# octavian-ganea/equidock_public

Hardware: NVIDIA H100
Metric: protein_pairs_per_sec_iegmn_fwd_kabsch (higher is better)
Workload: dtype f32

## Files before the change

### equidock_public_b200/csrc/attn_tc.cu

```cuda
#include "tc_common.cuh"

namespace eqd {

#define AT_THREADS 256
#define AT_KEYS 64
#define AT_CHUNK_BYTES 8192
#define AT_A_SPLIT 16384
#define AT_LD 68

struct AtGroupSmem {
  unsigned char k[2][3][AT_CHUNK_BYTES];
  unsigned char v[2][3][AT_CHUNK_BYTES];
  float red[EQD_TM * 2];
  float x5c[2][AT_KEYS * 16];
  float red5[EQD_TM * 2 * 5];
};
struct AtSmem {
  unsigned char qa[3 * AT_A_SPLIT];
  unsigned char pa[3 * AT_A_SPLIT];
  AtGroupSmem grp;
  unsigned long long k_bar[2], v_bar[2];
};

__global__ void __launch_bounds__(AT_THREADS, 1)
attention0_tc_kernel(eqd_graph g, const float* __restrict__ proj, int pw, const unsigned char* __restrict__ kv,
                    long kv_split_stride, const float* __restrict__ x5, float* __restrict__ mu, int ldmu) {
  extern __shared__ __align__(128) unsigned char smem_raw[];
  AtSmem& S = *reinterpret_cast<AtSmem*>(smem_raw);
  const int tid = threadIdx.x, q = tid, half = q >> 7, r = q & 127, wgi = tid >> 7;
  AtGroupSmem& G = S.grp;
  if (tid == 0) {
    for (int b = 0; b < 2; ++b) {
      mbar_init(&S.k_bar[b], 1);
      mbar_init(&S.v_bar[b], 1);
    }
    asm volatile("fence.mbarrier_init.release.cluster;" ::: "memory");
  }
  __syncthreads();
  const unsigned k_saddr = smem_u32(G.k), v_saddr = smem_u32(G.v);
  const unsigned qa_saddr = smem_u32(S.qa), pa_saddr = smem_u32(S.pa);
  float* const dtile = reinterpret_cast<float*>(S.pa);
  unsigned kph[2] = {0, 0}, vph[2] = {0, 0};
  const int B = g.n_pairs;
  const unsigned char* k_g = kv;
  const unsigned char* v_g = kv + 3 * kv_split_stride;

  auto load_chunk = [&](const unsigned char* src, unsigned char (*dst)[AT_CHUNK_BYTES], unsigned long long* bar, int blk0,
                        int x5buf) {
    if (q == 0) {
      const bool with5 = x5buf >= 0;
      mbar_expect_tx(bar, 3 * AT_CHUNK_BYTES + (with5 ? AT_KEYS * 64 : 0));
#pragma unroll
      for (int s = 0; s < 3; ++s) bulk_g2s(dst[s], src + s * kv_split_stride + (long)blk0 * 1024, AT_CHUNK_BYTES, bar);
      if (with5) bulk_g2s(G.x5c[x5buf], x5 + (long)blk0 * 8 * 16, AT_KEYS * 64, bar);
    }
  };
  auto add_s5 = [&](float (&s)[32], const float* xc, const float (&q5)[5]) {
#pragma unroll
    for (int i = 0; i < 32; ++i) {
      const float* row = xc + (half * 32 + i) * 16;
      const float4 k4 = *reinterpret_cast<const float4*>(row);
      const float k8 = row[8];
      s[i] += q5[0] * k4.x + q5[1] * k4.y + q5[2] * k4.z + q5[3] * k4.w + q5[4] * k8;
    }
  };
  auto gemm_s = [&](int kb_, bool hi_only) {
    float d[32];
    wg_gemm6<64>(d, [&](int sp, int kb) { return a_desc_at<EQD_TM>(qa_saddr, AT_A_SPLIT, wgi, sp, kb); },
                 [&](int sp, int kk) { return b_desc_ex(k_saddr + (kb_ * 3 + sp) * AT_CHUNK_BYTES + kk * 256, 128, 1024); },
                 4, false, hi_only);
    wg_store_d<64>(dtile + wgi * 64 * AT_LD, AT_LD, d, tid & 127);
  };
  auto gemm_pv = [&](int vb_) {
    float d[32];
    wg_gemm6<64, 1>(d, [&](int sp, int kb) { return a_desc_at<EQD_TM>(pa_saddr, AT_A_SPLIT, wgi, sp, kb); },
                    [&](int sp, int kk) { return b_desc_ex(v_saddr + (vb_ * 3 + sp) * AT_CHUNK_BYTES + kk * 2048, 1024, 128); },
                    4, false);
    __syncthreads();
    wg_store_d<64>(dtile + wgi * 64 * AT_LD, AT_LD, d, tid & 127);
  };

  for (int tile = blockIdx.x; tile < g.n_node_tiles; tile += gridDim.x) {
    const int seg = g.node_tiles[2 * tile], node0 = g.node_tiles[2 * tile + 1];
    const int nvalid = min(EQD_TM, g.seg_ptr[seg + 1] - node0);
    const int pseg = seg < B ? seg + B : seg - B;
    const int j0 = g.seg_ptr[pseg], j1 = g.seg_ptr[pseg + 1];
    const int blk_lo = j0 >> 3, blk_hi = (j1 + 7) >> 3;
    const int nchunks = (blk_hi - blk_lo + 7) >> 3;
    const int node = node0 + r;
    const bool valid = r < nvalid;
    if (nchunks > 0) load_chunk(k_g, G.k[0], &S.k_bar[0], blk_lo, 0);
    float q5[5] = {0.f, 0.f, 0.f, 0.f, 0.f};
    if (valid) {
#pragma unroll
      for (int e = 0; e < 5; ++e) q5[e] = x5[(long)node * 16 + 10 + e];
    }
    {
      float v[32];
      const float4* sp = reinterpret_cast<const float4*>(proj + (long)node * pw + 128 + half * 32);
#pragma unroll
      for (int c4 = 0; c4 < 8; ++c4) {
        float4 t = valid ? sp[c4] : make_float4(0.f, 0.f, 0.f, 0.f);
        v[c4 * 4] = t.x; v[c4 * 4 + 1] = t.y; v[c4 * 4 + 2] = t.z; v[c4 * 4 + 3] = t.w;
      }
      store_half_split3<EQD_TM>(S.qa, AT_A_SPLIT, r, half * 32, v);
    }
    tc_fence_before();
    __syncthreads();
    float mx = -INFINITY;
    for (int c = 0; c < nchunks; ++c) {
      const int kb_ = c & 1;
      mbar_wait(&S.k_bar[kb_], kph[kb_]);
      kph[kb_] ^= 1;
      if (c + 1 < nchunks) load_chunk(k_g, G.k[kb_ ^ 1], &S.k_bar[kb_ ^ 1], blk_lo + 8 * (c + 1), kb_ ^ 1);
      else load_chunk(k_g, G.k[kb_ ^ 1], &S.k_bar[kb_ ^ 1], blk_lo, kb_ ^ 1);
      gemm_s(kb_, true);
      __syncthreads();
      float s[32];
      tile_ld32f(dtile, AT_LD, r, half * 32, s);
      add_s5(s, G.x5c[kb_], q5);
      const int key0 = (blk_lo + 8 * c) * 8 + half * 32;
#pragma unroll
      for (int i = 0; i < 32; ++i) {
        int kn = key0 + i;
        mx = fmaxf(mx, (kn >= j0 && kn < j1) ? s[i] : -INFINITY);
      }
      __syncthreads();
    }
    G.red[r * 2 + half] = mx;
    __syncthreads();
    mx = fmaxf(G.red[r * 2], G.red[r * 2 + 1]);
    float l = 0.f;
    float o_acc[32];
#pragma unroll
    for (int i = 0; i < 32; ++i) o_acc[i] = 0.f;
    if (nchunks > 0) load_chunk(v_g, G.v[0], &S.v_bar[0], blk_lo, -1);
    float o5[5] = {0.f, 0.f, 0.f, 0.f, 0.f};
    for (int c = 0; c < nchunks; ++c) {
      const int kb_ = (nchunks + c) & 1, vb_ = c & 1;
      mbar_wait(&S.k_bar[kb_], kph[kb_]);
      kph[kb_] ^= 1;
      if (c + 1 < nchunks) {
        load_chunk(k_g, G.k[kb_ ^ 1], &S.k_bar[kb_ ^ 1], blk_lo + 8 * (c + 1), kb_ ^ 1);
        load_chunk(v_g, G.v[vb_ ^ 1], &S.v_bar[vb_ ^ 1], blk_lo + 8 * (c + 1), -1);
      }
      gemm_s(kb_, false);
      __syncthreads();
      float s[32];
      tile_ld32f(dtile, AT_LD, r, half * 32, s);
      add_s5(s, G.x5c[kb_], q5);
      const int key0 = (blk_lo + 8 * c) * 8 + half * 32;
      float l4[4] = {0.f, 0.f, 0.f, 0.f};
#pragma unroll
      for (int i = 0; i < 32; ++i) {
        int kn = key0 + i;
        float pj = (kn >= j0 && kn < j1) ? expf(s[i] - mx) : 0.f;
        s[i] = pj;
        l4[i & 3] += pj;
        {
          const float* row = G.x5c[kb_] + (half * 32 + i) * 16;
          const float4 v4 = *reinterpret_cast<const float4*>(row + 4);
          o5[0] = fmaf(pj, v4.x, o5[0]);
          o5[1] = fmaf(pj, v4.y, o5[1]);
          o5[2] = fmaf(pj, v4.z, o5[2]);
          o5[3] = fmaf(pj, v4.w, o5[3]);
          o5[4] = fmaf(pj, row[9], o5[4]);
        }
      }
      l += (l4[0] + l4[1]) + (l4[2] + l4[3]);
      __syncthreads();
      store_half_split3<EQD_TM>(S.pa, AT_A_SPLIT, r, half * 32, s);
      tc_fence_before();
      __syncthreads();
      mbar_wait(&S.v_bar[vb_], vph[vb_]);
      vph[vb_] ^= 1;
      gemm_pv(vb_);
      __syncthreads();
      {
        float oc[32];
        tile_ld32f(dtile, AT_LD, r, half * 32, oc);
#pragma unroll
        for (int i = 0; i < 32; ++i) o_acc[i] += oc[i];
      }
      __syncthreads();
    }
    G.red[r * 2 + half] = l;
    {
#pragma unroll
      for (int e = 0; e < 5; ++e) G.red5[(r * 2 + half) * 5 + e] = o5[e];
    }
    __syncthreads();
    l = G.red[r * 2] + G.red[r * 2 + 1];
    {
      const float inv = l > 0.f ? 1.f / l : 0.f;
      if (valid && half == 0) {
        float e8[8];
#pragma unroll
        for (int e = 0; e < 5; ++e) e8[e] = (G.red5[r * 10 + e] + G.red5[r * 10 + 5 + e]) * inv;
        e8[5] = e8[6] = e8[7] = 0.f;
        float4* de = reinterpret_cast<float4*>(mu + (long)node * ldmu + 64);
        de[0] = make_float4(e8[0], e8[1], e8[2], e8[3]);
        de[1] = make_float4(e8[4], e8[5], e8[6], e8[7]);
      }
      if (valid) {
        float4* dst = reinterpret_cast<float4*>(mu + (long)node * ldmu + half * 32);
#pragma unroll
        for (int c4 = 0; c4 < 8; ++c4)
          dst[c4] = make_float4(o_acc[c4 * 4] * inv, o_acc[c4 * 4 + 1] * inv, o_acc[c4 * 4 + 2] * inv, o_acc[c4 * 4 + 3] * inv);
      }
    }
    __syncthreads();
  }
}

#define AT_CHAINS 2

struct __align__(128) AtChainSmem {
  unsigned char k[2][3][AT_CHUNK_BYTES];
  unsigned char v[2][3][AT_CHUNK_BYTES];
  float qs[64 * 64];
  unsigned long long k_bar[2], v_bar[2];
};

struct AtTile {
  int node0, nvalid;
  int j0, j1;
  int blk_lo, nchunks;
};

template <int P>
__global__ void __launch_bounds__(AT_CHAINS * 128, 1)
attention64_tc_kernel(eqd_graph g, const float* __restrict__ proj, const unsigned char* __restrict__ kv,
                      long kv_split_stride, float* __restrict__ mu) {
  extern __shared__ __align__(128) unsigned char smem_raw[];
  AtChainSmem& W = reinterpret_cast<AtChainSmem*>(smem_raw)[threadIdx.x >> 7];
  const int tid = threadIdx.x, wgi = tid >> 7, t = tid & 127, lane = t & 31;
  const int bar = 1 + wgi;
  if (t == 0) {
    for (int b = 0; b < 2; ++b) {
      mbar_init(&W.k_bar[b], 1);
      mbar_init(&W.v_bar[b], 1);
    }
    asm volatile("fence.mbarrier_init.release.cluster;" ::: "memory");
  }
  wg_barrier(bar);
  const unsigned k_saddr = smem_u32(W.k), v_saddr = smem_u32(W.v);
  const int B = g.n_pairs, nht = 2 * g.n_node_tiles, hstride = gridDim.x * AT_CHAINS;
  const unsigned char* k_g = kv;
  const unsigned char* v_g = kv + 3 * kv_split_stride;

  const int chain = blockIdx.x * AT_CHAINS + wgi;
  auto find_tile = [&](int k, AtTile& m) {
    for (; chain + k * hstride < nht; ++k) {
      const int ht = (chain + k * hstride) ^ (k & 1);
      const int seg = __ldg(g.node_tiles + 2 * (ht >> 1));
      m.node0 = __ldg(g.node_tiles + 2 * (ht >> 1) + 1) + 64 * (ht & 1);
      m.nvalid = min(64, __ldg(g.seg_ptr + seg + 1) - m.node0);
      if (m.nvalid <= 0) continue;
      const int pseg = seg < B ? seg + B : seg - B;
      m.j0 = __ldg(g.seg_ptr + pseg);
      m.j1 = __ldg(g.seg_ptr + pseg + 1);
      m.blk_lo = m.j0 >> 3;
      m.nchunks = (((m.j1 + 7) >> 3) - m.blk_lo + 7) >> 3;
      return k;
    }
    return -1;
  };
  unsigned kfill = 0, kcons = 0, vfill = 0, vcons = 0;
  auto fill = [&](unsigned char (*dst)[3][AT_CHUNK_BYTES], unsigned long long* bars, unsigned& n, const unsigned char* src,
                  int blk0) {
    if (t == 0) {
      unsigned long long* b = &bars[n & 1];
      mbar_expect_tx(b, 3 * AT_CHUNK_BYTES);
#pragma unroll
      for (int s = 0; s < 3; ++s) bulk_g2s(dst[n & 1][s], src + s * kv_split_stride + (long)blk0 * 1024, AT_CHUNK_BYTES, b);
    }
    ++n;
  };
  auto consume = [&](unsigned long long* bars, unsigned& n) {
    mbar_wait(&bars[n & 1], (n >> 1) & 1);
    return (int)((n++) & 1);
  };
  auto stage_q = [&](const AtTile& m) { stage_rows64(W.qs, proj, 320, 128, m.node0, m.nvalid, t); };

  const int fr0 = (t >> 5) * 16 + (lane >> 2), fc = 2 * (lane & 3);
  AtTile cur, nxt;
  int kt = find_tile(0, cur);
  bool k_ahead = false, v_ahead = false;
  if (kt >= 0) stage_q(cur);
  while (kt >= 0) {
    int ktn = -1;
    bool looked = false;
    auto look_ahead = [&]() {
      if (looked) return;
      looked = true;
      ktn = find_tile(kt + 1, nxt);
      if (ktn >= 0) stage_q(nxt);
    };
    if (cur.nchunks > 0 && !k_ahead) fill(W.k, W.k_bar, kfill, k_g, cur.blk_lo);
    cp_async_wait<0>();
    wg_barrier(bar);
    unsigned qf[3][4][4];
    staged_rows_to_a_split3<P>(W.qs, t, qf);
    wg_barrier(bar);
    auto k_desc = [&](int kb_) {
      return [&, kb_](int sp, int kk) { return b_desc_ex(k_saddr + (kb_ * 3 + sp) * AT_CHUNK_BYTES + kk * 256, 128, 1024); };
    };
    float mx[2] = {-INFINITY, -INFINITY};
    for (int c = 0; c < cur.nchunks; ++c) {
      const int kb_ = consume(W.k_bar, kcons);
      fill(W.k, W.k_bar, kfill, k_g, cur.blk_lo + (c + 1 < cur.nchunks ? 8 * (c + 1) : 0));
      float s[32];
      wg_gemm6_rs_issue<64, 4, 0, true>(s, qf, k_desc(kb_), false);
      look_ahead();
      wg_mma_wait(s);
      const int key0 = (cur.blk_lo + 8 * c) * 8 + fc;
#pragma unroll
      for (int j = 0; j < 8; ++j)
#pragma unroll
        for (int e = 0; e < 2; ++e) {
          const int kn = key0 + 8 * j + e;
          const bool ok = kn >= cur.j0 && kn < cur.j1;
#pragma unroll
          for (int h = 0; h < 2; ++h) mx[h] = fmaxf(mx[h], ok ? s[4 * j + 2 * h + e] : -INFINITY);
        }
      wg_barrier(bar);
    }
    look_ahead();
#pragma unroll
    for (int h = 0; h < 2; ++h) {
      mx[h] = fmaxf(mx[h], __shfl_xor_sync(0xffffffffu, mx[h], 1));
      mx[h] = fmaxf(mx[h], __shfl_xor_sync(0xffffffffu, mx[h], 2));
    }
    float lh[2][2] = {{0.f, 0.f}, {0.f, 0.f}};
    float o_acc[32];
#pragma unroll
    for (int i = 0; i < 32; ++i) o_acc[i] = 0.f;
    if (cur.nchunks > 0 && !v_ahead) fill(W.v, W.v_bar, vfill, v_g, cur.blk_lo);
    for (int c = 0; c < cur.nchunks; ++c) {
      const int kb_ = consume(W.k_bar, kcons);
      const bool last = c + 1 == cur.nchunks;
      if (!last) {
        fill(W.k, W.k_bar, kfill, k_g, cur.blk_lo + 8 * (c + 1));
        fill(W.v, W.v_bar, vfill, v_g, cur.blk_lo + 8 * (c + 1));
      } else if (ktn >= 0 && nxt.nchunks > 0) {
        fill(W.k, W.k_bar, kfill, k_g, nxt.blk_lo);
        fill(W.v, W.v_bar, vfill, v_g, nxt.blk_lo);
      }
      float s[32];
      wg_gemm6_rs_issue<64, 4, 0, false, P>(s, qf, k_desc(kb_), false);
      wg_mma_wait(s);
      const int key0 = (cur.blk_lo + 8 * c) * 8 + fc;
#pragma unroll
      for (int j = 0; j < 8; ++j)
#pragma unroll
        for (int e = 0; e < 2; ++e) {
          const int kn = key0 + 8 * j + e;
          const bool ok = kn >= cur.j0 && kn < cur.j1;
#pragma unroll
          for (int h = 0; h < 2; ++h) {
            float& x = s[4 * j + 2 * h + e];
            x = ok ? expf(x - mx[h]) : 0.f;
          }
        }
      {
        float ps[32];
#pragma unroll
        for (int i = 0; i < 32; ++i) ps[i] = __shfl_xor_sync(0xffffffffu, s[i], 2);
#pragma unroll
        for (int h = 0; h < 2; ++h)
#pragma unroll
          for (int ch = 0; ch < 2; ++ch) {
            float s0 = 0.f, s1 = 0.f;
#pragma unroll
            for (int c4 = 0; c4 < 8; ++c4) {
              s0 = __fadd_rn(s0, chain_val(s, ps, h, ch, c4, 0));
              s1 = __fadd_rn(s1, chain_val(s, ps, h, ch, c4, 1));
            }
            const float sp = __fadd_rn(s0, s1);
            lh[h][ch] = __fadd_rn(lh[h][ch], __fadd_rn(sp, __shfl_xor_sync(0xffffffffu, sp, 1)));
          }
      }
      unsigned pf[3][4][4];
      acc_to_a_split3<4, P>(s, pf);
      const int vb_ = consume(W.v_bar, vcons);
      float o[32];
      wg_gemm6_rs_issue<64, 4, 1, false, P>(o, pf, [&](int sp, int kk) {
        return b_desc_ex(v_saddr + (vb_ * 3 + sp) * AT_CHUNK_BYTES + kk * 2048, 1024, 128); }, false);
      wg_mma_wait(o);
#pragma unroll
      for (int i = 0; i < 32; ++i) o_acc[i] = __fadd_rn(o_acc[i], o[i]);
      wg_barrier(bar);
    }
    k_ahead = v_ahead = ktn >= 0 && nxt.nchunks > 0 && cur.nchunks > 0;
#pragma unroll
    for (int h = 0; h < 2; ++h) {
      const float l = __fadd_rn(lh[h][0], lh[h][1]);
      const float inv = l > 0.f ? 1.f / l : 0.f;
      const int row = fr0 + 8 * h;
      if (row < cur.nvalid) {
        float* dst = mu + (long)(cur.node0 + row) * EQD_HID + fc;
#pragma unroll
        for (int j = 0; j < 8; ++j)
          *reinterpret_cast<float2*>(dst + 8 * j) = make_float2(o_acc[4 * j + 2 * h] * inv, o_acc[4 * j + 2 * h + 1] * inv);
      }
    }
    kt = ktn;
    cur = nxt;
  }
  cp_async_wait<0>();
}

template <int P>
static int launch_attention64_tc(const eqd_graph* g, const float* proj, const void* kv, float* mu, void* stream) {
  const size_t smem = AT_CHAINS * sizeof(AtChainSmem);
  EQD_SET_SMEM(attention64_tc_kernel<P>, smem);
  const int nht = 2 * g->n_node_tiles;
  int grid = (nht + AT_CHAINS - 1) / AT_CHAINS;
  if (grid > EQD_SMS) grid = EQD_SMS;
  const long split_stride = (long)((g->n_nodes + 7) / 8 + 8) * 1024;
  attention64_tc_kernel<P><<<grid, AT_CHAINS * 128, smem, (cudaStream_t)stream>>>(
      *g, proj, reinterpret_cast<const unsigned char*>(kv), split_stride, mu);
  EQD_CUDA_LAUNCH_CHECK();
  return EQD_OK;
}

}

int eqd_attention_tc_products(const eqd_graph* g, const float* proj, const void* kv, float* mu, int products, void* stream) {
  if (!g || !proj || !kv || !mu) return EQD_ERR_BAD_ARG;
  if (reinterpret_cast<uintptr_t>(kv) & 15) return EQD_ERR_BAD_ARG;
  if (products != 6 && products != 3) return EQD_ERR_UNSUPPORTED;
  if (g->n_node_tiles <= 0) return EQD_OK;
  return products == 3 ? eqd::launch_attention64_tc<3>(g, proj, kv, mu, stream)
                       : eqd::launch_attention64_tc<6>(g, proj, kv, mu, stream);
}

extern "C" int eqd_attention_tc(const eqd_graph* g, const float* proj, const void* kv, float* mu, void* stream) {
  return eqd_attention_tc_products(g, proj, kv, mu, 6, stream);
}

extern "C" int eqd_attention_tc0(const eqd_graph* g, const float* proj, const void* kv, const float* x5, float* mu,
                                 void* stream) {
  if (!g || !proj || !kv || !x5 || !mu) return EQD_ERR_BAD_ARG;
  if ((reinterpret_cast<uintptr_t>(kv) | reinterpret_cast<uintptr_t>(x5)) & 15) return EQD_ERR_BAD_ARG;
  if (g->n_node_tiles <= 0) return EQD_OK;
  const size_t smem = sizeof(eqd::AtSmem) + 128;
  EQD_SET_SMEM(eqd::attention0_tc_kernel, smem);
  const int grid = g->n_node_tiles < EQD_SMS ? g->n_node_tiles : EQD_SMS;
  const long split_stride = (long)((g->n_nodes + 7) / 8 + 8) * 1024;
  eqd::attention0_tc_kernel<<<grid, AT_THREADS, smem, (cudaStream_t)stream>>>(
      *g, proj, 128 + 3 * 72, reinterpret_cast<const unsigned char*>(kv), split_stride, x5, mu, EQD_H0_PAD);
  EQD_CUDA_LAUNCH_CHECK();
  return EQD_OK;
}
```

Measured before the change: 43090.

## Double-issue K chunks in max pass with per-slot barriers and single-plane K loads

```diff
diff --git a/equidock_public_b200/csrc/attn_tc.cu b/equidock_public_b200/csrc/attn_tc.cu
--- a/equidock_public_b200/csrc/attn_tc.cu
+++ b/equidock_public_b200/csrc/attn_tc.cu
@@ -219,7 +219,7 @@
   unsigned char k[2][3][AT_CHUNK_BYTES];
   unsigned char v[2][3][AT_CHUNK_BYTES];
   float qs[64 * 64];
-  unsigned long long k_bar[2], v_bar[2];
+  unsigned long long k_bar[6], v_bar[2];
 };
 
 struct AtTile {
@@ -237,10 +237,8 @@
   const int tid = threadIdx.x, wgi = tid >> 7, t = tid & 127, lane = t & 31;
   const int bar = 1 + wgi;
   if (t == 0) {
-    for (int b = 0; b < 2; ++b) {
-      mbar_init(&W.k_bar[b], 1);
-      mbar_init(&W.v_bar[b], 1);
-    }
+    for (int b = 0; b < 6; ++b) mbar_init(&W.k_bar[b], 1);
+    for (int b = 0; b < 2; ++b) mbar_init(&W.v_bar[b], 1);
     asm volatile("fence.mbarrier_init.release.cluster;" ::: "memory");
   }
   wg_barrier(bar);
@@ -266,20 +264,32 @@
     }
     return -1;
   };
-  unsigned kfill = 0, kcons = 0, vfill = 0, vcons = 0;
-  auto fill = [&](unsigned char (*dst)[3][AT_CHUNK_BYTES], unsigned long long* bars, unsigned& n, const unsigned char* src,
-                  int blk0) {
+  constexpr int NP = P == 6 ? 3 : 2;
+  auto fill = [&](unsigned char* dst, unsigned long long* b, const unsigned char* src, int blk0, int planes) {
     if (t == 0) {
-      unsigned long long* b = &bars[n & 1];
-      mbar_expect_tx(b, 3 * AT_CHUNK_BYTES);
-#pragma unroll
-      for (int s = 0; s < 3; ++s) bulk_g2s(dst[n & 1][s], src + s * kv_split_stride + (long)blk0 * 1024, AT_CHUNK_BYTES, b);
-    }
-    ++n;
-  };
-  auto consume = [&](unsigned long long* bars, unsigned& n) {
-    mbar_wait(&bars[n & 1], (n >> 1) & 1);
-    return (int)((n++) & 1);
+      mbar_expect_tx(b, planes * AT_CHUNK_BYTES);
+      for (int s = 0; s < planes; ++s)
+        bulk_g2s(dst + s * AT_CHUNK_BYTES, src + s * kv_split_stride + (long)blk0 * 1024, AT_CHUNK_BYTES, b);
+    }
+  };
+  int kh = 0;
+  unsigned kph = 0;
+  auto fill_k = [&](int slot, int blk0, int planes) { fill(W.k[0][0] + slot * AT_CHUNK_BYTES, &W.k_bar[slot], k_g, blk0, planes); };
+  auto wait_k = [&](int slot) {
+    mbar_wait(&W.k_bar[slot], (kph >> slot) & 1);
+    kph ^= 1u << slot;
+  };
+  auto k_desc = [&](int slot) {
+    return [&, slot](int sp, int kk) { return b_desc_ex(k_saddr + (slot + sp) * AT_CHUNK_BYTES + kk * 256, 128, 1024); };
+  };
+  unsigned vfill = 0, vcons = 0;
+  auto fill_v = [&](int blk0) {
+    fill(W.v[vfill & 1][0], &W.v_bar[vfill & 1], v_g, blk0, NP);
+    ++vfill;
+  };
+  auto consume_v = [&]() {
+    mbar_wait(&W.v_bar[vcons & 1], (vcons >> 1) & 1);
+    return (int)((vcons++) & 1);
   };
   auto stage_q = [&](const AtTile& m) { stage_rows64(W.qs, proj, 320, 128, m.node0, m.nvalid, t); };
 
@@ -289,6 +299,7 @@
   bool k_ahead = false, v_ahead = false;
   if (kt >= 0) stage_q(cur);
   while (kt >= 0) {
+    const int n = cur.nchunks;
     int ktn = -1;
     bool looked = false;
     auto look_ahead = [&]() {
@@ -297,23 +308,23 @@
       ktn = find_tile(kt + 1, nxt);
       if (ktn >= 0) stage_q(nxt);
     };
-    if (cur.nchunks > 0 && !k_ahead) fill(W.k, W.k_bar, kfill, k_g, cur.blk_lo);
+    auto kb2 = [&](int c) { return kh ^ 1 ^ (c & 1); };
+    if (n > 0 && !k_ahead) {
+      fill_k(3 * kh, cur.blk_lo, 1);
+      if (n > 1) fill_k(3 * kh + 1, cur.blk_lo + 8, 1);
+    }
     cp_async_wait<0>();
     wg_barrier(bar);
     unsigned qf[3][4][4];
     staged_rows_to_a_split3<P>(W.qs, t, qf);
     wg_barrier(bar);
-    auto k_desc = [&](int kb_) {
-      return [&, kb_](int sp, int kk) { return b_desc_ex(k_saddr + (kb_ * 3 + sp) * AT_CHUNK_BYTES + kk * 256, 128, 1024); };
+    float mx[2] = {-INFINITY, -INFINITY};
+    auto p1_issue = [&](float (&s)[32], int c) {
+      const int slot = 3 * kh + c % 3;
+      wait_k(slot);
+      wg_gemm6_rs_issue<64, 4, 0, true>(s, qf, k_desc(slot), false);
     };
-    float mx[2] = {-INFINITY, -INFINITY};
-    for (int c = 0; c < cur.nchunks; ++c) {
-      const int kb_ = consume(W.k_bar, kcons);
-      fill(W.k, W.k_bar, kfill, k_g, cur.blk_lo + (c + 1 < cur.nchunks ? 8 * (c + 1) : 0));
-      float s[32];
-      wg_gemm6_rs_issue<64, 4, 0, true>(s, qf, k_desc(kb_), false);
-      look_ahead();
-      wg_mma_wait(s);
+    auto p1_reduce = [&](const float (&s)[32], int c) {
       const int key0 = (cur.blk_lo + 8 * c) * 8 + fc;
 #pragma unroll
       for (int j = 0; j < 8; ++j)
@@ -325,8 +336,36 @@
           for (int h = 0; h < 2; ++h) mx[h] = fmaxf(mx[h], ok ? s[4 * j + 2 * h + e] : -INFINITY);
         }
       wg_barrier(bar);
-    }
-    look_ahead();
+    };
+    auto p1_fill = [&](int c) {
+      if (c + 2 < n) fill_k(3 * kh + (c + 2) % 3, cur.blk_lo + 8 * (c + 2), 1);
+      else if (c == max(n - 2, 0)) fill_k(3 * kb2(0), cur.blk_lo, NP);
+    };
+    auto p1_step = [&](float (&s)[32], float (&sn)[32], int c) {
+      p1_fill(c);
+      p1_issue(sn, c + 1);
+      wg_mma_wait<1>(s);
+      p1_reduce(s, c);
+    };
+    if (n > 0) {
+      float sa[32], sb[32];
+      p1_issue(sa, 0);
+      int c = 0;
+      for (; c + 2 < n; c += 2) {
+        p1_step(sa, sb, c);
+        p1_step(sb, sa, c + 1);
+      }
+      if (c + 1 < n) {
+        p1_step(sa, sb, c);
+        p1_fill(c + 1);
+        wg_mma_wait(sb);
+        p1_reduce(sb, c + 1);
+      } else {
+        p1_fill(c);
+        wg_mma_wait(sa);
+        p1_reduce(sa, c);
+      }
+    }
 #pragma unroll
     for (int h = 0; h < 2; ++h) {
       mx[h] = fmaxf(mx[h], __shfl_xor_sync(0xffffffffu, mx[h], 1));
@@ -336,19 +375,24 @@
     float o_acc[32];
 #pragma unroll
     for (int i = 0; i < 32; ++i) o_acc[i] = 0.f;
-    if (cur.nchunks > 0 && !v_ahead) fill(W.v, W.v_bar, vfill, v_g, cur.blk_lo);
-    for (int c = 0; c < cur.nchunks; ++c) {
-      const int kb_ = consume(W.k_bar, kcons);
-      const bool last = c + 1 == cur.nchunks;
+    if (n > 0 && !v_ahead) fill_v(cur.blk_lo);
+    for (int c = 0; c < n; ++c) {
+      const bool last = c + 1 == n;
       if (!last) {
-        fill(W.k, W.k_bar, kfill, k_g, cur.blk_lo + 8 * (c + 1));
-        fill(W.v, W.v_bar, vfill, v_g, cur.blk_lo + 8 * (c + 1));
-      } else if (ktn >= 0 && nxt.nchunks > 0) {
-        fill(W.k, W.k_bar, kfill, k_g, nxt.blk_lo);
-        fill(W.v, W.v_bar, vfill, v_g, nxt.blk_lo);
+        fill_k(3 * kb2(c + 1), cur.blk_lo + 8 * (c + 1), NP);
+        fill_v(cur.blk_lo + 8 * (c + 1));
+      } else {
+        look_ahead();
+        if (ktn >= 0 && nxt.nchunks > 0) {
+          fill_k(3 * (kb2(c) ^ 1), nxt.blk_lo, 1);
+          if (nxt.nchunks > 1) fill_k(3 * (kb2(c) ^ 1) + 1, nxt.blk_lo + 8, 1);
+          fill_v(nxt.blk_lo);
+        }
       }
       float s[32];
-      wg_gemm6_rs_issue<64, 4, 0, false, P>(s, qf, k_desc(kb_), false);
+      wait_k(3 * kb2(c));
+      wg_gemm6_rs_issue<64, 4, 0, false, P>(s, qf, k_desc(3 * kb2(c)), false);
+      look_ahead();
       wg_mma_wait(s);
       const int key0 = (cur.blk_lo + 8 * c) * 8 + fc;
 #pragma unroll
@@ -383,7 +427,7 @@
       }
       unsigned pf[3][4][4];
       acc_to_a_split3<4, P>(s, pf);
-      const int vb_ = consume(W.v_bar, vcons);
+      const int vb_ = consume_v();
       float o[32];
       wg_gemm6_rs_issue<64, 4, 1, false, P>(o, pf, [&](int sp, int kk) {
         return b_desc_ex(v_saddr + (vb_ * 3 + sp) * AT_CHUNK_BYTES + kk * 2048, 1024, 128); }, false);
@@ -392,7 +436,9 @@
       for (int i = 0; i < 32; ++i) o_acc[i] = __fadd_rn(o_acc[i], o[i]);
       wg_barrier(bar);
     }
-    k_ahead = v_ahead = ktn >= 0 && nxt.nchunks > 0 && cur.nchunks > 0;
+    look_ahead();
+    k_ahead = v_ahead = ktn >= 0 && nxt.nchunks > 0 && n > 0;
+    if (n > 0) kh ^= (n - 1) & 1;
 #pragma unroll
     for (int h = 0; h < 2; ++h) {
       const float l = __fadd_rn(lh[h][0], lh[h][1]);
```

After: 44140, median of 6. 1.02x the previous value.
